# coin-or/Ipopt

Measured on AMD Instinct MI355X. Metric: KKT factor+solve GFLOP/s (1 numeric LDL^T factorisation + 2 solves per Ipopt iteration), higher is better.
Workload: dtype f64; 1 GPU; synth_1e6; kkt_dim=1000000, triplet_nnz=20143342, nnz_L=230755000, ordering=nested dissection + minimum-degree leaves (own), supernodes=50052, tree_levels=110, maxfront=3260, num_neg=400000

## Files before the change

ipopt_amd/csrc/api.cpp:

```cpp
#include "../../include/mi355x_kkt.h"
#include "symbolic.h"
#include "numeric.h"
#include "launch_plan.h"
#include "matching_scaling.h"
#include "comm_shm.h"
#include "env_knobs.h"
#include <algorithm>
#include <cmath>
#include <cstdio>
#include <cstring>
#include <new>
#include <string>
#include <thread>
#include <chrono>
#include <vector>

using namespace mi355x;

struct mi355x_kkt_handle_s {
    mi355x_kkt_options opts;
    Symbolic sym;
    Numeric* num = nullptr;
    bool analysed = false, numeric_ready = false, factored = false;
    bool stats_stale = false;
// ... 435 lines not shown
        case 21: v = &S.dup_ptr; break;    case 22: v = &S.dup_src; break;    case 23: v = &S.sn_class; break;
        case 24: v = &S.rslot_ptr; break;  case 25: v = &S.rslot_idx; break;  case 26: v = &S.rslot_col; break;
        default: h->err = "get_symbolic: unknown selector"; return MI355X_KKT_FATAL;
    }
    if ((int64_t)v->size() > cap) { h->err = "get_symbolic: buffer too small"; return MI355X_KKT_FATAL; }
    if (!v->empty()) std::memcpy(out, v->data(), v->size() * sizeof(int));
    return MI355X_KKT_SUCCESS;
}

int mi355x_kkt_get_launch_plan(mi355x_kkt_handle h, int nranks, int rank, const char* what, int* out, int64_t cap, int64_t* count)
{
    if (!h || !what || !count) return MI355X_KKT_FATAL;
    if (!h->analysed) { h->err = "get_launch_plan: analyse() first"; return MI355X_KKT_FATAL; }
    if (nranks != std::max(1, h->so.nranks) || rank < 0 || rank >= nranks) { h->err = "get_launch_plan: nranks is the analysis's, 0 <= rank < nranks"; return MI355X_KKT_FATAL; }
    try {
        const LaunchPlan P = build_launch_plan(h->sym, plan_inputs_from_env(nranks, rank, nranks > 1, 0));
        if (!P.error.empty()) { h->err = P.error; return MI355X_KKT_FATAL; }
        std::vector<int> v;
        auto put = [&](std::initializer_list<long long> x) { for (long long e : x) v.push_back((int)e); };
        const std::string w(what);
        const Sched* sc = w.rfind("single.", 0) == 0 ? &P.single : w.rfind("local.", 0) == 0 ? &P.local : nullptr;
        if (w.rfind("stage", 0) == 0) { const int d = atoi(w.c_str() + 5); if (d >= 0 && d < (int)P.stage.size()) sc = &P.stage[d]; }
        const std::string field = sc ? w.substr(w.find('.') + 1) : w;
        if (sc) {
            if (field == "ptr") v = sc->ptr; else if (field == "base") put({sc->base}); else if (field == "maxm") v = sc->maxm; else if (field == "maxk") v = sc->maxk;
            else if (field == "last0") v = sc->last0; else if (field == "last1") v = sc->last1; else if (field == "allsolo") v.assign(sc->allsolo.begin(), sc->allsolo.end());
            else { h->err = "get_launch_plan: unknown schedule field"; return MI355X_KKT_FATAL; }
        } else if (w == "scalars") put({P.nlevels, P.ndepth, P.lc_levels, P.lc_nchains, P.la_any, P.grouped, P.ntfuse, P.nbig, (long long)P.stage.size()});
        else if (w == "level_list") v = P.lvl_list;
        else if (w == "tiny16") v = P.tiny16;
        else if (w == "tiny_split") v = P.tiny_split;
        else if (w == "mid_split") v = P.mid_split;
        else if (w == "big_split") v = P.big_split;
        else if (w == "lc_ptr") v = P.lc_ptr;
        else if (w == "lc_fronts") { for (const LeafLink& K : P.lc_link) v.push_back(K.s); if (P.lc_levels == 0) v.clear(); }
        else if (w == "df_runs") for (const DfRun& R : P.df_runs) put({R.lv0, R.lv1, R.tab0, R.nlev, R.nq});
        else if (w == "chain_segs") for (const ChainSeg& G : P.chain_segs) put({G.lv0, G.lv1, G.desc0, G.ndesc, G.nwg_f, G.nwg_b, G.maxtail, G.wgf0, G.wgb0});
        else if (w == "chain_links") for (const ChainLink& K : P.chl) put({K.s, K.k, K.koff, K.fi});
        else if (w == "chain_descs") for (const ChainDesc& D : P.chd) put({D.link0, D.nlinks, D.tail, D.ktot, D.s0, D.init});
        else if (w == "join") for (const JoinList& J : P.join) put({J.base, J.count, J.maxm, J.who});
        else if (w == "exchange") for (const RangeSeg& G : P.ex.rsegs) put({G.d, G.glo, G.gsz, G.aend - G.abeg, G.tend - G.tbeg});
        else if (w == "col_owner") v = P.col_owner;
        else if (w == "stat_owner") v = P.stat_owner;
        else { h->err = "get_launch_plan: unknown array"; return MI355X_KKT_FATAL; }
        *count = (int64_t)v.size();
        if (out) { if ((int64_t)v.size() > cap) { h->err = "get_launch_plan: buffer too small"; return MI355X_KKT_FATAL; } std::copy(v.begin(), v.end(), out); }
        return MI355X_KKT_SUCCESS;
    } catch (...) { h->err = "get_launch_plan: unexpected exception"; return MI355X_KKT_FATAL; }
}

int mi355x_kkt_profile(mi355x_kkt_handle h, int reps, double* ms, int* launches, int capacity)
{
    if (!h || !ms || !launches) return MI355X_KKT_FATAL;
    if (!h->numeric_ready || !h->factored) { h->err = "profile: factor() first"; return MI355X_KKT_FATAL; }
    if (capacity < MI355X_KKT_KERNEL_COUNT) { h->err = "profile: capacity too small"; return MI355X_KKT_FATAL; }
    try { if (!h->num->profile(reps > 0 ? reps : 1, ms, launches)) { h->err = h->num->error(); return MI355X_KKT_FATAL; } return MI355X_KKT_SUCCESS; }
    catch (...) { h->err = "profile: unexpected exception"; return MI355X_KKT_FATAL; }
}

int mi355x_kkt_debug_clocks(mi355x_kkt_handle h, unsigned long long* out128)
{
    if (!h || !h->numeric_ready) return MI355X_KKT_FATAL;
    try { return h->num->debug_clocks(out128) ? 0 : MI355X_KKT_FATAL; } catch (...) { return MI355X_KKT_FATAL; }
}

int mi355x_kkt_debug_pivots(mi355x_kkt_handle h, double* dinv, double* doff, int* ptype, int* lperm)
// ... 88 lines not shown
```

ipopt_amd/csrc/kernels_fronts.hip.inc:

```
template <int TS>
__device__ __forceinline__ void publish_col(double* buf, const double (&t)[TS][TS], const int row0, const int jl)
{
#pragma unroll
    for (int b = 0; b < TS; ++b)
        if (jl == b) {
#pragma unroll
            for (int a = 0; a < TS; ++a) { double v = t[a][b]; asm volatile("" : "+v"(v)); buf[row0 + a] = v; }
        }
}

#ifdef MI355X_PIVSTAT
__device__ unsigned long long g_fstat[32];
__device__ unsigned long long g_dt[16], g_dtacc[16];
__device__ unsigned long long g_pivstat[16];
#ifdef MI355X_PIVSTAT_COUNT
#define PIVSTAT(i) do { if (threadIdx.x == 0) atomicAdd(&g_pivstat[i], 1ull); } while (0)
#else
#define PIVSTAT(i) do { } while (0)
#endif
#else
#define PIVSTAT(i) do { } while (0)
#endif

__device__ __forceinline__ double fast_rcp(double d)
// ... 689 lines not shown
    }
#pragma unroll
    for (int sl = 0; sl < 2; ++sl) {
        const int r = wrow[sl];
        if (r >= 0 && r < m) {
#pragma unroll
            for (int g = 0; g < 4; ++g) { const int c = l4 + 4 * g; if (c < k) F[pk(r, c)] = wacc[sl][g]; }
        }
    }
    __syncthreads();
    {
        int q = 0;
        for (int tc = 0; tc < ntl; ++tc)
            for (int ti = max(tc, 1); ti < ntl; ++ti, ++q) {
                if ((q & 3) != wave) continue;
                v4f64_ acc = (v4f64_){0.0, 0.0, 0.0, 0.0};
                const int ri = 16 * ti + l15, rc = 16 * tc + l15;
#pragma unroll
                for (int t = 0; t < 4; ++t) {
                    const int p = 4 * t + l4;
                    const double av = (ri < m && p < k) ? F[pk(min(ri, m - 1), p)] * dinv_s[min(p, 15)] : 0.0;
                    const double bv = (rc < m && rc >= k && p < k) ? F[pk(min(max(rc, p), m - 1), p)] : 0.0;
                    acc = __builtin_amdgcn_mfma_f64_16x16x4f64(av, bv, acc, 0, 0, 0);
                }
                const int cc = 16 * tc + l15;
#pragma unroll
                for (int g = 0; g < 4; ++g) { const int rr = 16 * ti + l4 + 4 * g; if (rr < m && cc >= k && rr >= cc) F[pk(rr, cc)] -= acc[g]; }
            }
    }
    __syncthreads();
    return true;
}

template <int J> __device__ __forceinline__ void fast16_step_masked(double (&a)[16], double& rsave, const int l15, const bool on)
{
    const double t = a[J];
    const double d = bcast16<J>(t);
    const double ri = on ? fast_rcp(d) : 0.0;
    rsave = (on && l15 == J) ? ri : rsave;
    const double l = on ? t * ri : 0.0;
    rank1_dpp16<J>(a, t, l);
    a[J] = on ? l : t;
}
__device__ __forceinline__ void st_coh(double* p, double v);
__device__ __forceinline__ void st_coh(int* p, int v);
__device__ __forceinline__ void st_tagged(v2d* p, const double v, const double ep) { const v2d m = (v2d){v, ep}; asm volatile("global_store_dwordx4 %0, %1, off sc1" :: "v"(p), "v"(m) : "memory"); }
__device__ __forceinline__ void ld_tagged_row16(const v2d* p, v2d (&r)[16])
{
    asm volatile("global_load_dwordx4 %0, %16, off sc1\n\tglobal_load_dwordx4 %1, %16, off offset:256 sc1\n\tglobal_load_dwordx4 %2, %16, off offset:512 sc1\n\tglobal_load_dwordx4 %3, %16, off offset:768 sc1\n\t"
                 "global_load_dwordx4 %4, %16, off offset:1024 sc1\n\tglobal_load_dwordx4 %5, %16, off offset:1280 sc1\n\tglobal_load_dwordx4 %6, %16, off offset:1536 sc1\n\tglobal_load_dwordx4 %7, %16, off offset:1792 sc1\n\t"
                 "global_load_dwordx4 %8, %16, off offset:2048 sc1\n\tglobal_load_dwordx4 %9, %16, off offset:2304 sc1\n\tglobal_load_dwordx4 %10, %16, off offset:2560 sc1\n\tglobal_load_dwordx4 %11, %16, off offset:2816 sc1\n\t"
                 "global_load_dwordx4 %12, %16, off offset:3072 sc1\n\tglobal_load_dwordx4 %13, %16, off offset:3328 sc1\n\tglobal_load_dwordx4 %14, %16, off offset:3584 sc1\n\tglobal_load_dwordx4 %15, %16, off offset:3840 sc1\n\t"
                 "s_waitcnt vmcnt(0)"
                 : "=&v"(r[0]), "=&v"(r[1]), "=&v"(r[2]), "=&v"(r[3]), "=&v"(r[4]), "=&v"(r[5]), "=&v"(r[6]), "=&v"(r[7]), "=&v"(r[8]), "=&v"(r[9]), "=&v"(r[10]), "=&v"(r[11]), "=&v"(r[12]), "=&v"(r[13]), "=&v"(r[14]), "=&v"(r[15])
                 : "v"(p) : "memory");
}
__device__ __forceinline__ bool df_wait_expired(const DevView& V, const int spins)
{
    if (spins > (1 << 22) || ((spins & 1023) == 0 && __hip_atomic_load(&V.qstat[6], __ATOMIC_RELAXED, __HIP_MEMORY_SCOPE_AGENT) != 0)) { V.qstat[6] = 1; V.qstat[4] = 1; return true; }
    return false;
}
template <bool DF>
__device__ __forceinline__ void front_dpp16_body(const DevView& V, double (&Fs)[4][16 * 17], int (&relS)[4][16], const int list_off, const int nfronts, const int quad, const int top_mode, const int no_strict_behind, const int epoch)
{
    const int lane = threadIdx.x, g = lane >> 4, li = lane & 15;
    const int f = 4 * quad + g;
// ... 570 lines not shown
```

ipopt_amd/csrc/launch_plan.cpp:

```cpp
#include "launch_plan.h"
#include "env_knobs.h"
#include <algorithm>
#include <cstdio>
#include <map>

namespace mi355x {

PlanInputs plan_inputs_from_env(int nranks, int rank, bool multi, int verbose)
{
    PlanInputs in;
    in.nranks = nranks; in.rank = rank; in.multi = multi; in.verbose = verbose;
    in.chain_solve = !knob_disabled("chain_solve"); in.fuse_dt = !knob_disabled("fuse_dt"); in.fastpiv = !knob_disabled("fastpiv");
    in.asm_pull = !knob_disabled("asm_pull"); in.leafchain = !knob_disabled("leafchain"); in.front_df = !knob_disabled("front_df");
    in.tfuse = !knob_disabled("tfuse"); in.fuse_upd = !knob_disabled("fuse_upd"); in.selfasm = !knob_disabled("selfasm");
    in.grouped = !knob_disabled("grouped"); in.xcd_tiles = !knob_disabled("xcd_tiles"); in.lookahead = !knob_disabled("lookahead");
    in.pair_solve = !knob_disabled("pair_solve"); in.p1_small = !knob_disabled("p1_small");
    in.la_wgs = (int)std::max(1ll, knob_int("la_wgs", in.la_wgs));
    in.la_min_nt = (int)std::max(3ll, knob_int("la_min_nt", in.la_min_nt));
    in.la_min_tiles = knob_int("la_min_tiles", in.la_min_tiles);
    in.grp_rbw_max = (int)std::max(1ll, knob_int("grp_rbw_max", in.grp_rbw_max));
    in.chain_solve_maxc = (int)std::max(1ll, knob_int("chain_solve_maxc", in.chain_solve_maxc));
    in.fuse_dt_maxwg = (int)knob_int("fuse_dt_maxwg", in.fuse_dt_maxwg);
    knob_tune("fastpiv_floor", &in.fastpiv_floor);
    return in;
}

static int order_of(const Symbolic& Sy, int s) { return Sy.sn_rowptr[s + 1] - Sy.sn_rowptr[s]; }
static int cols_of(const Symbolic& Sy, int s) { return Sy.sn_colptr[s + 1] - Sy.sn_colptr[s]; }
static int nchild(const Symbolic& Sy, int s) { return Sy.child_ptr[s + 1] - Sy.child_ptr[s]; }
static int tri_tiles(int nt) { const int t = nt * (nt + 1) / 2; return nt >= 12 ? (t + 7) / 8 * 8 : t; }
static int schur_tiles64(const Symbolic& Sy, int s)
{
    const int nt = (order_of(Sy, s) - cols_of(Sy, s) + 63) / 64;
    return Sy.grp_rem[s] > 0 ? nt * ((Sy.grp_rem[s] + 63) / 64) : nt * (nt + 1) / 2;
}
static int schur_tiles(const Symbolic& Sy, int s)
{
    const int nt = (order_of(Sy, s) - cols_of(Sy, s) + 127) / 128;
    return Sy.grp_rem[s] > 0 ? nt * ((Sy.grp_rem[s] + 127) / 128) : tri_tiles(nt);
}
static size_t front_lds(size_t m, size_t k, size_t maxm)
{
    const size_t ld = m | 1, ldi = k | 1;
    return (std::max(m * (m + 1) / 2, k * ld + k * ldi) + 4 * maxm + 3 * k) * sizeof(double) + 2 * k * sizeof(int) + 64;
}
static bool same_range(const Symbolic& Sy, int a, int b) { return Sy.sn_owner[a] < 0 && Sy.sn_owner[b] < 0 && Sy.sn_glo[a] == Sy.sn_glo[b] && Sy.sn_gsz[a] == Sy.sn_gsz[b]; }
static bool crosses(const Symbolic& Sy, int c) { const int pa = Sy.sn_parent[c]; return pa >= 0 && Sy.sn_owner[pa] < 0 && !same_range(Sy, c, pa); }

ExchangeLayout exchange_layout(const Symbolic& Sy, int ndepth)
// ... 23 lines not shown
        }
        X.aend[d] = X.arena_doubles; X.tend[d] = X.toprhs_doubles;
    }
    return X;
}

void comm_plan(const Symbolic& Sy, int nranks, int rank, bool range_local, std::vector<int>& out)
{
    const int ndepth = std::max(1, Sy.num_gdepths);
    const ExchangeLayout X = exchange_layout(Sy, ndepth);
    auto rec = [&](int what, int d, int colour, int gsz, long long count, int dtype) { out.push_back(what); out.push_back(d); out.push_back(colour); out.push_back(gsz); out.push_back((int)std::min<long long>(count, 0x7fffffffll)); out.push_back(dtype); };
    if (range_local)
        for (int d = 0; d < ndepth; ++d) {
            bool partial = false; int color = -1;
            for (const RangeSeg& sg : X.rsegs) if (sg.d == d && sg.gsz < nranks) { partial = true; if (sg.glo <= rank && rank < sg.glo + sg.gsz) color = sg.glo; }
            if (partial) rec(0, d, color, 0, 0, 1);
        }
    auto step = [&](int d, int what) {
        if (range_local) {
            for (const RangeSeg& sg : X.rsegs) {
                if (sg.d != d || !(sg.glo <= rank && rank < sg.glo + sg.gsz)) continue;
                const long long cnt = what == 1 ? sg.aend - sg.abeg : sg.tend - sg.tbeg;
                if (cnt > 0) rec(what, d, sg.gsz >= nranks ? -2 : sg.glo, sg.gsz, cnt, 0);
            }
        } else {
            const long long cnt = what == 1 ? X.aend[d] - X.abeg[d] : X.tend[d] - X.tbeg[d];
            if (cnt > 0) rec(what, d, -2, nranks, cnt, 0);
        }
    };
    for (int d = ndepth - 1; d >= 0; --d) step(d, 1);
    rec(2, 0, -2, nranks, 8, 1);
    for (int d = ndepth - 1; d >= 0; --d) step(d, 3);
    if (Sy.n > 0) rec(4, 0, -2, nranks, Sy.n, 0);
}

LaunchPlan build_launch_plan(const Symbolic& Sy, const PlanInputs& in)
{
    LaunchPlan P;
    const int NL = Sy.num_levels, NS = Sy.num_sn;
    const bool multi = in.multi;
    P.nlevels = NL;
    auto bucket0 = [&](int lv, int fc) { return Sy.level_ptr[(size_t)lv * FC_COUNT + fc]; };
    auto pool_remap = [&](long long lin) {
        if (in.pool_cut.empty()) return lin;
        const size_t i = (size_t)(std::upper_bound(in.pool_cut.begin(), in.pool_cut.end(), lin) - in.pool_cut.begin()) - 1; return lin + in.pool_delta[i]; };
    P.panel_off.resize(NS); P.cb_off.resize(NS);
    for (int sn = 0; sn < NS; ++sn) {
        P.panel_off[sn] = pool_remap(Sy.panel_off[sn]);
        P.cb_off[sn] = pool_remap(Sy.l_doubles + Sy.cb_off[sn]) - Sy.l_doubles;
    }
    std::vector<int>& L = P.lvl_list;
    L.assign(Sy.level_sn.begin(), Sy.level_sn.end());
    std::vector<char> solve_entry;
    auto in_sched = [&](int which, int s) {
        if (which == 0) return true;
        if (which == 1) return Sy.sn_owner[s] == in.rank;
        return Sy.sn_owner[s] < 0 && Sy.sn_glo[s] <= in.rank && in.rank < Sy.sn_glo[s] + Sy.sn_gsz[s] && Sy.sn_gdepth[s] == which - 2;
    };
    auto build_sched = [&](Sched& sc, int which) {
        sc.ptr.assign((size_t)NL * FC_COUNT + 1, 0); sc.base = which == 0 ? 0 : (int)L.size();
        sc.maxm.assign(NL, 0); sc.maxk.assign(NL, 0); sc.tiles.assign(NL, 0); sc.tiles64.assign(NL, 0);
        std::vector<std::vector<int>> bucket((size_t)NL * FC_COUNT);
        for (int s = 0; s < NS; ++s) {
            if (!in_sched(which, s)) continue;
            const int lv = Sy.sn_level[s];
            bucket[(size_t)lv * FC_COUNT + Sy.sn_class[s]].push_back(s);
// ... 250 lines not shown
    auto build_groups = [&](GrpSched& G, int which) {
        for (auto* v : {&G.g0, &G.g1, &G.split, &G.nrb, &G.tiles64, &G.tiles, &G.la1, &G.la2, &G.p1t, &G.la3, &G.nsplit}) v->assign(NL, 0);
        if (!P.grouped) return;
        std::vector<std::vector<int>> at(NL);
        for (int sn = 0; sn < NS; ++sn) if (Sy.sn_class[sn] == FC_BIG && Sy.grp_rem[sn] == 0 && in_sched(which, sn)) {
            int first = sn;
            for (int j = Sy.grp_pos[sn]; j > 0; --j) first = Sy.alias_child[first];
            if (Sy.sn_level[first] >= Sy.grp_cut_level) at[Sy.sn_level[first]].push_back(sn);
        }
        int ng = 0;
        for (int lv = 0; lv < NL; ++lv) {
            std::stable_sort(at[lv].begin(), at[lv].end(), [&](int a, int b) { return order_of(Sy, a) < order_of(Sy, b); });
            G.g0[lv] = (int)L.size();
            int nsmall = 0;
            for (int sn : at[lv]) {
                L.push_back(sn); ++ng;
                const int mu = upd_rows(sn), nt = (mu + 127) / 128;
                G.nrb[lv] = std::max(G.nrb[lv], (mu + 63) / 64);
                if (order_of(Sy, sn) <= 1024) { ++nsmall; G.tiles64[lv] = std::max(G.tiles64[lv], schur_tiles64(Sy, sn)); continue; }
                G.tiles[lv] = std::max(G.tiles[lv], schur_tiles(Sy, sn));
                G.la1[lv] = std::max(G.la1[lv], split_of[sn] ? 2 * nt - 1 : tri_tiles(nt));
                if (split_of[sn]) {
                    G.la2[lv] = std::max(G.la2[lv], ((nt - 2) * (nt - 1) / 2 + 7) / 8 * 8);
                    const int n64 = (mu + 63) / 64; int c = 0; for (int tc = 0; tc < 4 && tc < n64; ++tc) c += n64 - tc; G.p1t[lv] = std::max(G.p1t[lv], c); ++G.nsplit[lv];
                } else G.la3[lv] = std::max(G.la3[lv], tri_tiles(nt));
            }
            G.split[lv] = nsmall; G.g1[lv] = (int)L.size();
        }
        if (in.verbose) fprintf(stderr, "[mi355x_kkt] grouped schedule%s: %d chain groups factored in one launch each (tree levels >= %d)\n",
                                which == 0 ? "" : (which == 1 ? " (own subtrees)" : " (replicated fronts of one exchange step)"), ng, Sy.grp_cut_level);
    };
    P.grp.assign(multi ? 1 + P.ndepth : 1, GrpSched());
    for (size_t i = 0; i < P.grp.size(); ++i) build_groups(P.grp[i], multi ? 1 + (int)i : 0);
    std::vector<char> tfuse_of(NS, 0);
    std::vector<int> asmcut_of(NS, 0);
    if (!multi && in.tfuse)
        for (int sn = 0; sn < NS; ++sn) {
            if (Sy.sn_class[sn] != FC_BIG || Sy.grp_rem[sn] != 0) continue;
            int first = sn;
            for (int j = 0; j < Sy.grp_pos[sn]; ++j) first = Sy.alias_child[first];
            if (Sy.alias_child[first] >= 0 || upd_rows(sn) <= 0 || nchild(Sy, first) > 96) continue;
            tfuse_of[sn] = 1; ++P.ntfuse;
            asmcut_of[first] = order_of(Sy, first) - upd_rows(sn);
        }
    if (in.verbose) fprintf(stderr, "[mi355x_kkt] contribution blocks formed by their update (not assembled): %d of %d big fronts\n", P.ntfuse, Sy.num_big);
    P.fmeta.resize(L.size()); P.asm_fast_ok.assign(L.size(), 0); P.asmcut.assign(L.size(), 0);
    for (size_t q = 0; q < L.size(); ++q) {
        const int sn = L[q];
        FrontMeta& M = P.fmeta[q];
        int nside = 0;
        for (int c = Sy.child_ptr[sn]; c < Sy.child_ptr[sn + 1]; ++c) if (Sy.child_idx[c] != Sy.alias_child[sn]) ++nside;
        P.asm_fast_ok[q] = (Sy.alias_child[sn] >= 0 && nside == 0) ? 1 : (Sy.alias_child[sn] < 0 ? (nside <= 6 ? std::max(nside, 1) : 0) : 0);
        M.tfuse = tfuse_of[sn]; M.asmcut = asmcut_of[sn];
        M.s = sn; M.c0 = Sy.sn_colptr[sn]; M.k = cols_of(Sy, sn); M.r0 = Sy.sn_rowptr[sn]; M.m = order_of(Sy, sn);
        M.aq0 = Sy.acolptr[M.c0]; M.aq1 = Sy.acolptr[M.c0 + M.k]; M.ch0 = Sy.child_ptr[sn]; M.ch1 = Sy.child_ptr[sn + 1]; M.alias = Sy.alias_child[sn] >= 0 ? 1 : 0;
        M.ldp = Sy.sn_ldp[sn]; M.ldt = Sy.sn_ldt[sn];
        M.panel_off = P.panel_off[sn]; M.cb_off = P.cb_off[sn]; M.minv_off = Sy.minv_off[sn];
        M.cv = Sy.cv_off[sn]; M.wb = Sy.wb_off[sn]; M.gpart = Sy.gpart_off[sn];
        M.gbase = gbase_of[sn]; M.gpos = Sy.grp_pos[sn]; M.grem = Sy.grp_rem[sn]; M.gcols = gcols_of[sn]; M.split = split_of[sn]; M.ttab = ttab_of[sn]; M.ttab2 = ttab2_of[sn];
        M.selfasm = (Sy.sn_class[sn] == FC_BIG && selfasm(sn)) ? 1 : 0; M.bigidx = bigidx_of[sn];
        M.solo = (Sy.alias_child[sn] >= 0 && nchild(Sy, sn) == 1) ? 1 : ((Sy.alias_child[sn] < 0 && nchild(Sy, sn) == 0) ? 2 : 0);
        P.asmcut[q] = (M.selfasm && !M.asmcut) ? -1 : M.asmcut;
        if (q < solve_entry.size() && solve_entry[q] && !Sy.solve_group) {
            M.gbase += M.gpos; M.gpos = 0; M.grem = 0; M.gcols = M.k;
        }
    }
// ... 97 lines not shown
```

ipopt_amd/csrc/launch_plan.h:

```cpp
#pragma once
#include "symbolic.h"
#include "kernel_tables.h"
#include <cstddef>
#include <string>
#include <vector>

namespace mi355x {

struct PlanInputs {
    int nranks = 1, rank = 0;
    bool multi = false;
    int verbose = 0;
    bool chain_solve = true, fuse_dt = true, fastpiv = true, asm_pull = true, leafchain = true, front_df = true, tfuse = true, fuse_upd = true,
         selfasm = true, grouped = true, xcd_tiles = true, lookahead = true, pair_solve = true, p1_small = true;
    int la_wgs = 1 << 20, la_min_nt = 8, grp_rbw_max = 8, chain_solve_maxc = 128, fuse_dt_maxwg = 448;
    long long la_min_tiles = 4000;
    double fastpiv_floor = 1e-4;
    std::vector<long long> pool_cut, pool_delta;
};
PlanInputs plan_inputs_from_env(int nranks, int rank, bool multi, int verbose);

struct Sched { std::vector<int> ptr; int base = 0; std::vector<int> maxm, maxk, tiles, tiles64, last0, last1; std::vector<char> allsolo; };
struct GrpSched { std::vector<int> g0, g1, split, nrb, tiles64, tiles, la1, la2, p1t, la3, nsplit; };
struct ChainSeg { int lv0, lv1, desc0, ndesc, nwg_f, nwg_b, maxtail, wgf0, wgb0; };
struct JoinList { int base = 0, count = 0, maxm = 0, who = -1; };
struct RangeSeg { int d, glo, gsz; long long abeg, aend, tbeg, tend; };
struct DfRun { int lv0, lv1, tab0, nlev, nq; };

struct ExchangeLayout {
    std::vector<long long> aoff, troff;
    std::vector<long long> abeg, aend, tbeg, tend;
    std::vector<RangeSeg> rsegs;
    long long arena_doubles = 0, toprhs_doubles = 0;
};
ExchangeLayout exchange_layout(const Symbolic& Sy, int ndepth);
void comm_plan(const Symbolic& S, int nranks, int rank, bool range_local, std::vector<int>& out6);

struct LaunchPlan {
    int nlevels = 0;
    std::vector<int> lvl_list;
    Sched single;
    int ndepth = 1;
    Sched local; std::vector<Sched> stage;
    std::vector<JoinList> join;
    ExchangeLayout ex;
    std::vector<int> tiny16, tiny_split, mid_split, big_split, part_tiles[2];
    std::vector<size_t> mid_lds, reg_lds;
    std::vector<int> wave_kmax, wave_mmax, wave_mmin;
    bool pair_solve = true;
    std::vector<ChainSeg> chain_segs; std::vector<int> seg_at_lv0, seg_at_lv1;
    std::vector<char> in_seg;
    std::vector<ChainLink> chl; std::vector<ChainDesc> chd; std::vector<int> chwait, wgf, wgb;
    int ntailflags = 0, ndots = 0;
    std::vector<int> la_tiles1, la_tiles2; std::vector<char> la_full;
    bool la_any = false;
    std::vector<int> tile_tab;
    std::vector<char> lv_asm_skip;
    std::vector<int> lv_narrow_tiles;
    bool grouped = false;
    std::vector<GrpSched> grp;
    std::vector<char> asm_fast_ok; std::vector<int> asmcut;
    int ntfuse = 0, nbig = 0;
    std::string error;
    int lc_levels = 0, lc_nchains = 0;
    std::vector<int> lc_ptr; std::vector<LeafLink> lc_link;
    std::vector<DfRun> df_runs; std::vector<int> df_run_at; std::vector<DfLevel> df_tab; std::vector<long long> cbt_off; long long cbt_len = 0;
    std::vector<FrontMeta> fmeta; std::vector<ChildMeta> cmeta; std::vector<GroupLink> gtab; std::vector<int> relinv;
    std::vector<long long> panel_off, cb_off;
    std::vector<int> stat_owner, col_owner;
};
LaunchPlan build_launch_plan(const Symbolic& Sy, const PlanInputs& in);

}
```

ipopt_amd/csrc/numeric.hip:

```cpp
#include <hip/hip_runtime.h>
#include <rccl/rccl.h>
#include <dlfcn.h>
#include <cstdio>
#include <cstring>
#include <cmath>
#include <chrono>
#include <vector>
#include <thread>
#include <map>
#include <string>
#include <algorithm>
#include "numeric.h"
#include "launch_plan.h"
#include "env_knobs.h"
#include "matching_scaling.h"

namespace mi355x {

#define HIPCHK(call) do { hipError_t e_ = (call); if (e_ != hipSuccess) { \
    err_ = std::string(#call) + ": " + hipGetErrorString(e_); return false; } } while (0)

enum KernelKind { KK_GATHER_SCALE = 0, KK_FRONT_WAVE, KK_FRONT_LDS64, KK_FRONT_LDS128, KK_BIG_ASSEMBLE, KK_BIG_DIAG, KK_BIG_TRSM,
                  KK_BIG_SCHUR, KK_STATS, KK_SOLVE_PERM, KK_FWD_WAVE, KK_FWD_LDS, KK_FWD_BIG, KK_BWD_WAVE, KK_BWD_LDS, KK_BWD_BIG, KK_FWD_BIG_UPD, KK_BWD_BIG_DOT, KK_COUNT };
#define DBGSTAMP(slot) do { if (V.dbg && blockIdx.x == 0 && blockIdx.y == 0 && threadIdx.x == 0) { V.dbg[2 * (slot)] = clock64(); V.dbg[2 * (slot) + 1] = wall_clock64(); } } while (0)
// ... 551 lines not shown
        V.tvals = tv;
        V.rslot_len = (int)Sy.rslot_idx.size();
        if (!dalloc(&V.arv, Sy.rslot_idx.size()) || !dalloc(&V.aval, Sy.nnz_a) || !dalloc(&V.scale, Sy.n) || !dalloc(&V.scale2, Sy.n) || !dalloc(&V.rowmax, Sy.n) ||
            !dalloc(&V.wbuf, (size_t)Sy.wbuf_doubles) || !dalloc(&V.minv, (size_t)Sy.minv_doubles) ||
            !dalloc(&V.dinv, Sy.n) || !dalloc(&V.doff, Sy.n) || !dalloc(&V.ptype, Sy.n) || !dalloc(&V.lperm, Sy.n) ||
            !dalloc(&V.fstat, Sy.num_sn) || !dalloc(&V.xw, Sy.n) || !dalloc(&V.ybuf, Sy.n) || !dalloc(&V.zb, Sy.n) || !dalloc(&V.bw, Sy.n) || !dalloc(&V.xacc, Sy.n) || !dalloc(&V.cvec, (size_t)Sy.cvec_doubles) || !dalloc(&V.gpart, (size_t)Sy.gpart_doubles) ||
            !dalloc(&d_stats, 12) || !dalloc(&V.colfail, Sy.n) || !dalloc(&V.zpiv, Sy.n) || !dalloc(&V.cnorm, Sy.n) ||
            !dalloc(&V.sflag_d, Sy.num_sn) || !dalloc(&V.sflag_p, Sy.num_sn) || !dalloc(&V.sflag_s, 4 * (size_t)Sy.num_sn) || !dalloc(&V.tcnt, Sy.num_sn) || !dalloc(&V.apfail, Sy.num_sn) || !dalloc(&V.sepoch, 4)) return false;
        V.qstat = d_stats + 4;
        lap("device allocations");
        if (opt.scaling >= 3 && !d_user_scale) { HIPCHK(hipMalloc((void**)&d_user_scale, std::max<size_t>(Sy.n, 1) * sizeof(double))); allocs.push_back(d_user_scale); }
        else if (opt.scaling == 2 && !d_user_scale) opt.scaling = 1;
        V.cb = V.L + Sy.l_doubles;
        V.arena = nullptr; V.top_rhs = nullptr; V.rank = opt.rank; V.dbg = nullptr;
        if (knob_trace("clocks")) { if (!dalloc(&V.dbg, 128)) return false; }
        if (multi) { if (!dalloc(&V.arena, (size_t)P.ex.arena_doubles) || !dalloc(&V.top_rhs, (size_t)P.ex.toprhs_doubles)) return false; }
        V.pivtol = opt.pivtol; V.pivtol2 = std::max(opt.pivtol, opt.pivtolmax); V.small = opt.small; V.n = Sy.n; V.nnz_a = Sy.nnz_a; V.nsn = Sy.num_sn; V.xcd_affine = knob_disabled("xcd_affine") ? 0 : 1;
        la_ev.assign(1 + P.grp.size(), LaEvents());
        for (size_t i = 0; i < la_ev.size(); ++i) {
            const std::vector<int>& la2 = i == 0 ? P.la_tiles2 : P.grp[i - 1].la2;
            la_ev[i].A.assign(la2.size(), nullptr); la_ev[i].B.assign(la2.size(), nullptr);
            for (size_t lv = 0; lv < la2.size(); ++lv) if (la2[lv] > 0) {
                HIPCHK(hipEventCreateWithFlags(&la_ev[i].A[lv], hipEventDisableTiming)); HIPCHK(hipEventCreateWithFlags(&la_ev[i].B[lv], hipEventDisableTiming)); }
        }
        HIPCHK(hipFuncSetAttribute((const void*)k_big_diag_reg<4>, hipFuncAttributeMaxDynamicSharedMemorySize, 160 * 1024));
        HIPCHK(hipFuncSetAttribute((const void*)(k_big_diag_reg<4, 1024>), hipFuncAttributeMaxDynamicSharedMemorySize, 160 * 1024));
        HIPCHK(hipFuncSetAttribute((const void*)(k_front_reg<64, 2>), hipFuncAttributeMaxDynamicSharedMemorySize, 160 * 1024));
        HIPCHK(hipFuncSetAttribute((const void*)(k_front_reg<64, 4>), hipFuncAttributeMaxDynamicSharedMemorySize, 160 * 1024));
        HIPCHK(hipFuncSetAttribute((const void*)(k_front_reg<64, 8>), hipFuncAttributeMaxDynamicSharedMemorySize, 160 * 1024));
        HIPCHK(hipFuncSetAttribute((const void*)(k_front_reg<256, 8>), hipFuncAttributeMaxDynamicSharedMemorySize, 160 * 1024));
        HIPCHK(hipFuncSetAttribute((const void*)(k_front_reg<256, 6>), hipFuncAttributeMaxDynamicSharedMemorySize, 160 * 1024));
        HIPCHK(hipFuncSetAttribute((const void*)(k_front_reg<256, 8, true>), hipFuncAttributeMaxDynamicSharedMemorySize, 160 * 1024));
        HIPCHK(hipFuncSetAttribute((const void*)(k_front_reg<256, 6, true, 4>), hipFuncAttributeMaxDynamicSharedMemorySize, 160 * 1024));
        HIPCHK(hipFuncSetAttribute((const void*)k_big_trsm<false>, hipFuncAttributeMaxDynamicSharedMemorySize, 160 * 1024));
        HIPCHK(hipFuncSetAttribute((const void*)k_big_trsm<true>, hipFuncAttributeMaxDynamicSharedMemorySize, 160 * 1024));
        HIPCHK(hipFuncSetAttribute((const void*)k_big_diag_trsm, hipFuncAttributeMaxDynamicSharedMemorySize, 160 * 1024));
        HIPCHK(hipFuncSetAttribute((const void*)k_grp_fused, hipFuncAttributeMaxDynamicSharedMemorySize, 160 * 1024));
        HIPCHK(hipFuncSetAttribute((const void*)k_big_assemble2, hipFuncAttributeMaxDynamicSharedMemorySize, 158 * 1024));
        HIPCHK(hipDeviceSynchronize());
        lap("kernel attributes, zero fills landed");
        ready = true;
        if (keep && comm_kind == 2) make_subcomms();
        return true;
    }

    static size_t trsm_lds(int kk) { return trsm_lds_bytes(kk, false); }
    static int schur_grid(int tiles) { return SCHUR_GM == 2 ? 16 * ((tiles + 7) / 8) : tiles; }
    int grid1d(long long n) const { long long g = (n + 255) / 256; return (int)std::min<long long>(std::max<long long>(g, 1), 2048); }


    bool launch_bucket(int lv, int fc, int b0, int b1, int top_mode, int mm, int kk, int tiles, int tiles64) {
        const int nb = b1 - b0;
        const size_t rl = P.reg_lds[(size_t)lv * FC_COUNT + fc];
        if (fc == FC_WAVE) {
            const bool sg = b0 == S->level_ptr[(size_t)lv * FC_COUNT + FC_WAVE];
            const int nt = sg ? P.tiny_split[lv] : 0;
            int fl = top_mode;
            if (V.fastpiv && P.wave_mmin[lv] <= 16) {
                const int n16 = sg ? P.tiny16[lv] : nb;
                if (n16 > 0) { LAUNCH(KK_FRONT_WAVE, k_front_dpp16, dim3((n16 + 3) / 4), dim3(64), 0, stream, V, b0, n16, top_mode, (optimistic && n16 == nb) ? 1 : 0); fl |= 2; }
                if (optimistic && n16 == nb) return true;
            }
            if (nt > 0) LAUNCH(KK_FRONT_WAVE, (k_front_reg<64, 2>), dim3(nt), dim3(64), rl, stream, V, b0, fl);
            if (nb - nt > 0) LAUNCH(KK_FRONT_WAVE, (k_front_reg<64, 4>), dim3(nb - nt), dim3(64), rl, stream, V, b0 + nt, fl);
        } else if (fc == FC_LDS64) {
            LAUNCH(KK_FRONT_LDS64, (k_front_reg<64, 8>), dim3(nb), dim3(64), rl, stream, V, b0, top_mode);
        } else if (fc == FC_LDS128) {
            const int nm = (b0 == S->level_ptr[(size_t)lv * FC_COUNT + FC_LDS128]) ? P.mid_split[lv] : 0;
            const int fl = top_mode | (V.fastpiv ? 2 : 0);
            if (V.fastpiv) {
                if (nm > 0) LAUNCH(KK_FRONT_LDS128, (k_front_reg<256, 6, true, 4>), dim3(nm), dim3(256), P.mid_lds[lv], stream, V, b0, top_mode);
                if (nb - nm > 0) LAUNCH(KK_FRONT_LDS128, (k_front_reg<256, 8, true>), dim3(nb - nm), dim3(256), rl, stream, V, b0 + nm, top_mode);
            }
            if (nm > 0) LAUNCH(KK_FRONT_LDS128, (k_front_reg<256, 6>), dim3(nm), dim3(256), P.mid_lds[lv], stream, V, b0, fl);
            if (nb - nm > 0) LAUNCH(KK_FRONT_LDS128, (k_front_reg<256, 8>), dim3(nb - nm), dim3(256), rl, stream, V, b0 + nm, fl);
        } else {
            const bool single = (b0 == S->level_ptr[(size_t)lv * FC_COUNT + FC_BIG]) && !multi;
            if ((single || multi) && P.grouped && lv >= S->grp_cut_level) {
                if (!(single && P.lv_asm_skip[lv])) launch_assemble(mm, nb, b0, top_mode);
                return launch_groups(lv, top_mode ? 1 + grp_step : 0);
            }
            if (!single) { const bool sm = mm <= 640; return launch_big(lv, b0, sm ? b1 : b0, b1, top_mode, mm, kk, sm ? tiles64 : 0, sm ? 0 : tiles, false); }
            return launch_big(lv, b0, b0 + P.big_split[lv], b1, top_mode, mm, kk, P.part_tiles[0][lv], P.part_tiles[1][lv], true);
        }
        return true;
    }
    bool launch_groups(int lv, int gi) {
        const GrpSched& G = P.grp[gi]; const LaEvents& E = la_ev[1 + gi];
        const int b0 = G.g0[lv], b1 = G.g1[lv], bs = b0 + G.split[lv];
        if (b1 == b0) return true;
        {
            int rbw = 1;
            while (rbw < knobs.grp_rbw_max && (b1 - b0) * (4 + (G.nrb[lv] + rbw - 1) / rbw) > 256) rbw *= 2;
            const int nrbw = (G.nrb[lv] + rbw - 1) / rbw;
            const int st = ((b1 - b0) * (4 + nrbw) <= 256) ? 1 : 0;
            const size_t lds = std::max(diag_lds_bytes(64, 64), GRP_DB_BYTES + trsm_lds_bytes(64, st != 0));
            LAUNCH(KK_BIG_DIAG, k_grp_fused, dim3(b1 - b0, 4 + nrbw), dim3(256), lds, stream, V, b0, st, rbw, 0);
        }
        if (bs > b0 && G.tiles64[lv] > 0) LAUNCH(KK_BIG_SCHUR, k_big_schur64, dim3(G.tiles64[lv], bs - b0), dim3(256), 0, stream, V, b0, 0);
        if (b1 == bs) return true;
        const int nb = b1 - bs;
        if (la_pending) { HIPCHK(hipStreamWaitEvent(stream, la_last, 0)); la_pending = false; }
        if (G.la2[lv] > 0) {
            if (knobs.p1_small && G.la1[lv] * nb <= 512) {
                LAUNCH(KK_BIG_SCHUR, k_big_schur_p1, dim3(G.p1t[lv], nb), dim3(1024), 0, stream, V, bs);
                if (G.nsplit[lv] < nb) LAUNCH(KK_BIG_SCHUR, k_big_schur, dim3(schur_grid(G.la3[lv]), nb), dim3(SCHUR_NT), 0, stream, V, bs, 4, 0, 0);
            } else LAUNCH(KK_BIG_SCHUR, k_big_schur, dim3(schur_grid(G.la1[lv]), nb), dim3(SCHUR_NT), 0, stream, V, bs, 1, 0, 0);
            HIPCHK(hipEventRecord(E.A[lv], stream));
            HIPCHK(hipStreamWaitEvent(stream2, E.A[lv], 0));
            launch_part2(bs, nb, G.la2[lv]);
            HIPCHK(hipEventRecord(E.B[lv], stream2));
            la_last = E.B[lv]; la_pending = true;
        } else if (G.tiles[lv] > 0) LAUNCH(KK_BIG_SCHUR, k_big_schur, dim3(schur_grid(G.tiles[lv]), nb), dim3(SCHUR_NT), 0, stream, V, bs, 0, 0, 0);
// ... 947 lines not shown
```

Before: 9733 GFLOP/s.

## Add single-workgroup LDS-resident front kernel for small big-class supernodes

Adds k_front_wg, a 512-thread kernel that assembles, factors (16-column MFMA blocks with pivot checks), writes L/contribution blocks and inverts the diagonal block of a FC_BIG front entirely in LDS. The launch plan partitions each level's big fronts into eligible ones (order up to 192, at most 64 columns, not aliased or grouped), which use this kernel, and the rest, which stay on the multi-kernel big path. The aim is to cut launches and global round-trips for small big-class fronts. The cost is a new code path gated on the optimistic mode, packed-triangular LDS indexing, and another kernel whose numerics must match the existing path.

```diff
diff --git a/ipopt_amd/csrc/api.cpp b/ipopt_amd/csrc/api.cpp
--- a/ipopt_amd/csrc/api.cpp
+++ b/ipopt_amd/csrc/api.cpp
@@ -491,6 +491,7 @@
         else if (w == "tiny_split") v = P.tiny_split;
         else if (w == "mid_split") v = P.mid_split;
         else if (w == "big_split") v = P.big_split;
+        else if (w == "front_wg") for (int lv = 0; lv < P.nlevels; ++lv) put({P.wg0[lv], P.wg1[lv], P.rest0[lv], P.rest1[lv], P.rest_split[lv], P.wg_maxm[lv], P.wg_maxk[lv]});
         else if (w == "lc_ptr") v = P.lc_ptr;
         else if (w == "lc_fronts") { for (const LeafLink& K : P.lc_link) v.push_back(K.s); if (P.lc_levels == 0) v.clear(); }
         else if (w == "df_runs") for (const DfRun& R : P.df_runs) put({R.lv0, R.lv1, R.tab0, R.nlev, R.nq});
diff --git a/ipopt_amd/csrc/kernels_fronts.hip.inc b/ipopt_amd/csrc/kernels_fronts.hip.inc
--- a/ipopt_amd/csrc/kernels_fronts.hip.inc
+++ b/ipopt_amd/csrc/kernels_fronts.hip.inc
@@ -745,6 +745,186 @@
     return true;
 }
 
+constexpr int FRONT_WG_NT = 512;
+static size_t front_wg_lds_bytes(size_t m, size_t k) { return (std::max(m * (m + 1) / 2, k * (k | 1)) + 272 + 128) * sizeof(double) + 16; }
+template <int NT>
+__global__ __launch_bounds__(NT) void k_front_wg(DevView V, int list_off)
+{
+    extern __shared__ __attribute__((aligned(16))) char smem_raw[];
+    constexpr int NW = NT / 64;
+    const int tid = threadIdx.x, lane = tid & 63, wave = tid >> 6, l15 = lane & 15, l4 = lane >> 4;
+    const FrontMeta M = V.fmeta[list_off + blockIdx.x];
+    const int s = M.s, c0 = M.c0, k = M.k, m = M.m;
+    const int npk = m * (m + 1) / 2, ldi = k | 1;
+    double* F      = reinterpret_cast<double*>(smem_raw);
+    double* Xs     = F + max(npk, k * ldi);
+    double* dinv_s = Xs + 272;
+    double* cmv    = dinv_s + 64;
+    int*    shflag = reinterpret_cast<int*>(cmv + 64);
+    auto pk = [m](int i, int c) { return c * m - ((c * (c - 1)) >> 1) + (i - c); };
+    for (int idx = tid; idx < npk; idx += NT) F[idx] = 0.0;
+    if (tid == 0) { shflag[0] = 0; shflag[1] = 0; }
+    __syncthreads();
+    for (int q = M.aq0 + tid; q < M.aq1; q += NT) { const int pos = V.apos[q]; const int i = pos % m, c = pos / m; F[pk(i, c)] += V.aval[q]; }
+    __syncthreads();
+    {
+        int* relS = reinterpret_cast<int*>(Xs);
+        for (int cp = M.ch0; cp < M.ch1; ++cp) {
+            const ChildMeta* Cp = V.cmeta + cp;
+            const int mc = Cp->mc, ldt = Cp->ldt;
+            const double* C = V.cb + Cp->cb_off;
+            const int* relg = V.rel + Cp->relbase;
+            const unsigned d = (unsigned)(mc + 1), inv = 0xFFFFFFFFu / d + 1u;
+            const int npr = (mc + 1) >> 1, total = npr * (mc + 1);
+            for (int a = tid; a < mc; a += NT) relS[a] = relg[a];
+            auto decode = [&](int e, int& a, int& b) -> bool {
+                const int pr = (int)__umulhi((unsigned)e, inv), q = e - pr * (mc + 1);
+                const bool second = q >= mc - pr;
+                b = second ? mc - 1 - pr : pr;
+                a = second ? b + (q - (mc - pr)) : pr + q;
+                return e < total && !(second && 2 * pr == mc - 1);
+            };
+            __syncthreads();
+            constexpr int U = 8;
+            for (int base = 0; base < total; base += NT * U) {
+                double cvv[U];
+#pragma unroll
+                for (int u = 0; u < U; ++u) { int a, b; cvv[u] = decode(base + tid + NT * u, a, b) ? C[a + (size_t)b * ldt] : 0.0; }
+#pragma unroll
+                for (int u = 0; u < U; ++u) { int a, b; if (decode(base + tid + NT * u, a, b)) F[pk(relS[a], relS[b])] += cvv[u]; }
+            }
+            __syncthreads();
+        }
+    }
+    for (int c = tid >> 4; c < 64; c += NT / 16) {
+        const int part = tid & 15;
+        double mx = 0.0;
+        if (c < k) for (int i = part; i < m; i += 16) mx = fmax(mx, fabs(F[pk(max(i, c), min(i, c))]));
+        mx = fmax(mx, dpp_f64<0xB1>(mx)); mx = fmax(mx, dpp_f64<0x4E>(mx)); mx = fmax(mx, dpp_f64<0x141>(mx)); mx = fmax(mx, dpp_f64<0x140>(mx));
+        if (part == 0) cmv[c] = (c < k) ? fmax(mx, V.cnorm[c0 + c]) : 0.0;
+    }
+    __syncthreads();
+    const double cmx = wave_max_all(cmv[lane]);
+    const double zmax = fmax(V.small, ZERO_REL * cmx);
+    const double gmax = 1.0 / fmax(fmax(V.pivtol, V.pivtol2), V.fastu);
+    const int nbk = (k + 15) >> 4, ntl = (m + 15) >> 4;
+    int neg = 0;
+    bool ok = true;
+    for (int b = 0; b < nbk && ok; ++b) {
+        const int c16 = 16 * b, kb = min(16, k - c16);
+        if (wave == 0) {
+            const int row = c16 + l15;
+            double a[16], w[16], rsave = 1.0;
+#pragma unroll
+            for (int c = 0; c < 16; ++c) {
+                const int rr = min(row, m - 1), cc = min(c16 + c, m - 1);
+                const double v = F[pk(max(rr, cc), min(rr, cc))];
+                a[c] = (row < m && c16 + c < m) ? v : ((l15 == c) ? 1.0 : 0.0);
+                w[c] = 0.0;
+            }
+            asm volatile("s_waitcnt lgkmcnt(0)" ::: "memory");
+#define MI_STEP(j) if (j < kb) fast16_step<j>(a, w, rsave, l15);
+            MI_STEP(0) MI_STEP(1) MI_STEP(2) MI_STEP(3) MI_STEP(4) MI_STEP(5) MI_STEP(6) MI_STEP(7)
+            MI_STEP(8) MI_STEP(9) MI_STEP(10) MI_STEP(11) MI_STEP(12) MI_STEP(13) MI_STEP(14) MI_STEP(15)
+#undef MI_STEP
+            double gm = 0.0;
+#pragma unroll
+            for (int c = 0; c < 15; ++c) gm = fmax(gm, (c < kb && l15 > c) ? fabs(a[c]) : 0.0);
+            const bool mine = l15 < kb;
+            bool bad = __ballot(gm > gmax) != 0ull;
+            bad |= __ballot(mine && !(fabs(rsave) * zmax < 1.0)) != 0ull;
+            neg += __popcll(__ballot(mine && l4 == 0 && rsave < 0.0));
+            double x[4];
+#pragma unroll
+            for (int q = 0; q < 4; ++q) x[q] = (l15 == 4 * q + l4) ? 1.0 : 0.0;
+#define MI_INV(j) if (j + 1 < kb) fast16_inv<j>(a, x, l15, kb);
+            MI_INV(0) MI_INV(1) MI_INV(2) MI_INV(3) MI_INV(4) MI_INV(5) MI_INV(6) MI_INV(7) MI_INV(8) MI_INV(9) MI_INV(10) MI_INV(11) MI_INV(12) MI_INV(13) MI_INV(14)
+#undef MI_INV
+            if (bad) { if (lane == 0) shflag[0] = 1; }
+            else {
+#pragma unroll
+                for (int q = 0; q < 4; ++q) Xs[l15 + (4 * q + l4) * 17] = x[q];
+                if (l4 == 0 && mine) dinv_s[row] = rsave;
+                if (lane == 0) shflag[1] = neg;
+                if (l4 == 0 && row < m) {
+#pragma unroll
+                    for (int c = 0; c < 16; ++c) {
+                        if (c < kb) { if (l15 > c) F[pk(row, c16 + c)] = w[c]; }
+                        else if (l15 >= c) F[pk(row, c16 + c)] = a[c];
+                    }
+                }
+            }
+        }
+        __syncthreads();
+        if (shflag[0]) { ok = false; break; }
+        {
+            bool big = false;
+            for (int t = b + 1 + wave; t < ntl; t += NW) {
+                const int r = 16 * t + l15;
+                v4f64_ acc = (v4f64_){0.0, 0.0, 0.0, 0.0};
+#pragma unroll
+                for (int u = 0; u < 4; ++u) {
+                    const int p = 4 * u + l4;
+                    const double av = (p < kb && l15 < kb) ? Xs[l15 + p * 17] : 0.0;
+                    const double bv = (r < m && p < kb) ? F[pk(min(r, m - 1), c16 + min(p, kb - 1))] : 0.0;
+                    acc = __builtin_amdgcn_mfma_f64_16x16x4f64(av, bv, acc, 0, 0, 0);
+                }
+#pragma unroll
+                for (int g = 0; g < 4; ++g) {
+                    const int c = l4 + 4 * g;
+                    if (c < kb && r < m) { big |= fabs(acc[g] * dinv_s[c16 + c]) > gmax; F[pk(r, c16 + c)] = acc[g]; }
+                }
+            }
+            if (__ballot(big) != 0ull && lane == 0) shflag[0] = 1;
+        }
+        __syncthreads();
+        if (shflag[0]) { ok = false; break; }
+        {
+            int q = 0;
+            for (int tc = (kb == 16) ? b + 1 : b; tc < ntl; ++tc)
+                for (int ti = max(tc, b + 1); ti < ntl; ++ti, ++q) {
+                    if (q % NW != wave) continue;
+                    v4f64_ acc = (v4f64_){0.0, 0.0, 0.0, 0.0};
+                    const int ri = 16 * ti + l15, rc = 16 * tc + l15;
+#pragma unroll
+                    for (int t = 0; t < 4; ++t) {
+                        const int p = 4 * t + l4, col = c16 + min(p, kb - 1);
+                        const double av = (ri < m && p < kb) ? F[pk(min(ri, m - 1), col)] * dinv_s[col] : 0.0;
+                        const double bv = (rc < m && rc >= c16 + kb && p < kb) ? F[pk(min(max(rc, col), m - 1), col)] : 0.0;
+                        acc = __builtin_amdgcn_mfma_f64_16x16x4f64(av, bv, acc, 0, 0, 0);
+                    }
+                    const int cc = 16 * tc + l15;
+#pragma unroll
+                    for (int g = 0; g < 4; ++g) { const int rr = 16 * ti + l4 + 4 * g; if (rr < m && cc >= c16 + kb && rr >= cc) F[pk(rr, cc)] -= acc[g]; }
+                }
+        }
+        __syncthreads();
+    }
+    if (!ok) { if (tid == 0) { V.fstat[s] = make_int4(0, 0, 0, 0); V.qstat[4] = 1; } return; }
+    double* Lg = V.L + M.panel_off;
+    const size_t ldp = (size_t)M.ldp, ldt = (size_t)M.ldt;
+    for (int c = wave; c < k; c += NW) {
+        const double di = dinv_s[c];
+        for (int i = lane; i < m; i += 64) Lg[i + (size_t)c * ldp] = (i > c) ? F[pk(i, c)] * di : 0.0;
+    }
+    for (int jj = tid; jj < k; jj += NT) { V.dinv[c0 + jj] = dinv_s[jj]; V.doff[c0 + jj] = 0.0; V.ptype[c0 + jj] = 1; V.lperm[c0 + jj] = jj; }
+    double* Cg = V.cb + M.cb_off;
+    for (int c = k + wave; c < m; c += NW)
+        for (int i = c + lane; i < m; i += 64) Cg[(i - k) + (size_t)(c - k) * ldt] = F[pk(i, c)];
+    if (tid == 0) { V.fstat[s] = make_int4(shflag[1], 0, 0, 0); atomicAdd(&V.qstat[3], 1); }
+    constexpr int E = 4096 / NT;
+    double tmp[E];
+#pragma unroll
+    for (int e = 0; e < E; ++e) { const int idx = tid + e * NT; const int i = idx % k, c = idx / k; tmp[e] = (idx < k * k && i > c) ? F[pk(i, c)] * dinv_s[c] : 0.0; }
+    __syncthreads();
+#pragma unroll
+    for (int e = 0; e < E; ++e) { const int idx = tid + e * NT; const int i = idx % k, c = idx / k; if (idx < k * k) F[i + c * ldi] = tmp[e]; }
+    __syncthreads();
+    invert_unit_lower<NT>(F, ldi, k);
+    double* Mg = V.minv + M.minv_off;
+    for (int idx = tid; idx < k * k; idx += NT) { const int i = idx % k, c = idx / k; Mg[idx] = (i > c) ? F[i + c * ldi] : (i == c ? 1.0 : 0.0); }
+}
+
 template <int J> __device__ __forceinline__ void fast16_step_masked(double (&a)[16], double& rsave, const int l15, const bool on)
 {
     const double t = a[J];
diff --git a/ipopt_amd/csrc/launch_plan.cpp b/ipopt_amd/csrc/launch_plan.cpp
--- a/ipopt_amd/csrc/launch_plan.cpp
+++ b/ipopt_amd/csrc/launch_plan.cpp
@@ -14,7 +14,9 @@
     in.asm_pull = !knob_disabled("asm_pull"); in.leafchain = !knob_disabled("leafchain"); in.front_df = !knob_disabled("front_df");
     in.tfuse = !knob_disabled("tfuse"); in.fuse_upd = !knob_disabled("fuse_upd"); in.selfasm = !knob_disabled("selfasm");
     in.grouped = !knob_disabled("grouped"); in.xcd_tiles = !knob_disabled("xcd_tiles"); in.lookahead = !knob_disabled("lookahead");
-    in.pair_solve = !knob_disabled("pair_solve"); in.p1_small = !knob_disabled("p1_small");
+    in.pair_solve = !knob_disabled("pair_solve"); in.p1_small = !knob_disabled("p1_small"); in.front_wg = !knob_disabled("front_wg");
+    in.front_wg_partial = knob_int("front_wg_partial", in.front_wg_partial ? 1 : 0) != 0;
+    in.front_wg_maxm = (int)std::min<long long>(FRONT_WG_MAXM, std::max(0ll, knob_int("front_wg_maxm", in.front_wg_maxm)));
     in.la_wgs = (int)std::max(1ll, knob_int("la_wgs", in.la_wgs));
     in.la_min_nt = (int)std::max(3ll, knob_int("la_min_nt", in.la_min_nt));
     in.la_min_tiles = knob_int("la_min_tiles", in.la_min_tiles);
@@ -104,6 +106,12 @@
     rec(2, 0, -2, nranks, 8, 1);
     for (int d = ndepth - 1; d >= 0; --d) step(d, 3);
     if (Sy.n > 0) rec(4, 0, -2, nranks, Sy.n, 0);
+}
+
+bool front_wg_eligible(const Symbolic& Sy, int sn, int maxm)
+{
+    return Sy.sn_class[sn] == FC_BIG && order_of(Sy, sn) <= maxm && cols_of(Sy, sn) <= FRONT_WG_MAXK &&
+           Sy.alias_child[sn] < 0 && Sy.grp_pos[sn] == 0 && Sy.grp_rem[sn] == 0;
 }
 
 LaunchPlan build_launch_plan(const Symbolic& Sy, const PlanInputs& in)
@@ -420,6 +428,21 @@
     };
     P.grp.assign(multi ? 1 + P.ndepth : 1, GrpSched());
     for (size_t i = 0; i < P.grp.size(); ++i) build_groups(P.grp[i], multi ? 1 + (int)i : 0);
+    for (auto* v : {&P.wg0, &P.wg1, &P.wg_maxm, &P.wg_maxk, &P.rest0, &P.rest1, &P.rest_split, &P.rest_tiles[0], &P.rest_tiles[1]}) v->assign(NL, 0);
+    for (int lv = 0; lv < NL && !multi && in.front_wg; ++lv) {
+        if (P.grouped && lv >= Sy.grp_cut_level) continue;
+        std::vector<int> wg, rest;
+        for (int q = bucket0(lv, FC_BIG); q < bucket0(lv, FC_BIG + 1); ++q) (front_wg_eligible(Sy, L[q], in.front_wg_maxm) ? wg : rest).push_back(L[q]);
+        if (wg.empty() || (!rest.empty() && !in.front_wg_partial)) continue;
+        P.wg0[lv] = (int)L.size(); L.insert(L.end(), wg.begin(), wg.end()); P.wg1[lv] = (int)L.size();
+        for (int sn : wg) { P.wg_maxm[lv] = std::max(P.wg_maxm[lv], order_of(Sy, sn)); P.wg_maxk[lv] = std::max(P.wg_maxk[lv], cols_of(Sy, sn)); }
+        P.rest0[lv] = (int)L.size(); L.insert(L.end(), rest.begin(), rest.end()); P.rest1[lv] = (int)L.size();
+        for (int sn : rest) {
+            const int h = order_of(Sy, sn) <= 1024 ? 0 : 1;
+            if (h == 0) ++P.rest_split[lv];
+            P.rest_tiles[h][lv] = std::max(P.rest_tiles[h][lv], h == 0 ? schur_tiles64(Sy, sn) : schur_tiles(Sy, sn));
+        }
+    }
     std::vector<char> tfuse_of(NS, 0);
     std::vector<int> asmcut_of(NS, 0);
     if (!multi && in.tfuse)
diff --git a/ipopt_amd/csrc/launch_plan.h b/ipopt_amd/csrc/launch_plan.h
--- a/ipopt_amd/csrc/launch_plan.h
+++ b/ipopt_amd/csrc/launch_plan.h
@@ -12,8 +12,10 @@
     bool multi = false;
     int verbose = 0;
     bool chain_solve = true, fuse_dt = true, fastpiv = true, asm_pull = true, leafchain = true, front_df = true, tfuse = true, fuse_upd = true,
-         selfasm = true, grouped = true, xcd_tiles = true, lookahead = true, pair_solve = true, p1_small = true;
+         selfasm = true, grouped = true, xcd_tiles = true, lookahead = true, pair_solve = true, p1_small = true, front_wg = true;
     int la_wgs = 1 << 20, la_min_nt = 8, grp_rbw_max = 8, chain_solve_maxc = 128, fuse_dt_maxwg = 448;
+    bool front_wg_partial = true;
+    int front_wg_maxm = 192;
     long long la_min_tiles = 4000;
     double fastpiv_floor = 1e-4;
     std::vector<long long> pool_cut, pool_delta;
@@ -36,6 +38,9 @@
 ExchangeLayout exchange_layout(const Symbolic& Sy, int ndepth);
 void comm_plan(const Symbolic& S, int nranks, int rank, bool range_local, std::vector<int>& out6);
 
+constexpr int FRONT_WG_MAXM = 192, FRONT_WG_MAXK = 64;
+bool front_wg_eligible(const Symbolic& Sy, int sn, int maxm);
+
 struct LaunchPlan {
     int nlevels = 0;
     std::vector<int> lvl_list;
@@ -45,6 +50,7 @@
     std::vector<JoinList> join;
     ExchangeLayout ex;
     std::vector<int> tiny16, tiny_split, mid_split, big_split, part_tiles[2];
+    std::vector<int> wg0, wg1, wg_maxm, wg_maxk, rest0, rest1, rest_split, rest_tiles[2];
     std::vector<size_t> mid_lds, reg_lds;
     std::vector<int> wave_kmax, wave_mmax, wave_mmin;
     bool pair_solve = true;
diff --git a/ipopt_amd/csrc/numeric.hip b/ipopt_amd/csrc/numeric.hip
--- a/ipopt_amd/csrc/numeric.hip
+++ b/ipopt_amd/csrc/numeric.hip
@@ -607,6 +607,7 @@
         HIPCHK(hipFuncSetAttribute((const void*)(k_front_reg<256, 6>), hipFuncAttributeMaxDynamicSharedMemorySize, 160 * 1024));
         HIPCHK(hipFuncSetAttribute((const void*)(k_front_reg<256, 8, true>), hipFuncAttributeMaxDynamicSharedMemorySize, 160 * 1024));
         HIPCHK(hipFuncSetAttribute((const void*)(k_front_reg<256, 6, true, 4>), hipFuncAttributeMaxDynamicSharedMemorySize, 160 * 1024));
+        HIPCHK(hipFuncSetAttribute((const void*)k_front_wg<FRONT_WG_NT>, hipFuncAttributeMaxDynamicSharedMemorySize, 160 * 1024));
         HIPCHK(hipFuncSetAttribute((const void*)k_big_trsm<false>, hipFuncAttributeMaxDynamicSharedMemorySize, 160 * 1024));
         HIPCHK(hipFuncSetAttribute((const void*)k_big_trsm<true>, hipFuncAttributeMaxDynamicSharedMemorySize, 160 * 1024));
         HIPCHK(hipFuncSetAttribute((const void*)k_big_diag_trsm, hipFuncAttributeMaxDynamicSharedMemorySize, 160 * 1024));
@@ -654,6 +655,11 @@
             if ((single || multi) && P.grouped && lv >= S->grp_cut_level) {
                 if (!(single && P.lv_asm_skip[lv])) launch_assemble(mm, nb, b0, top_mode);
                 return launch_groups(lv, top_mode ? 1 + grp_step : 0);
+            }
+            if (single && optimistic && P.wg1[lv] > P.wg0[lv]) {
+                LAUNCH(KK_BIG_DIAG, k_front_wg<FRONT_WG_NT>, dim3(P.wg1[lv] - P.wg0[lv]), dim3(FRONT_WG_NT), front_wg_lds_bytes(P.wg_maxm[lv], P.wg_maxk[lv]), stream, V, P.wg0[lv]);
+                if (P.rest1[lv] == P.rest0[lv]) return true;
+                return launch_big(lv, P.rest0[lv], P.rest0[lv] + P.rest_split[lv], P.rest1[lv], top_mode, mm, kk, P.rest_tiles[0][lv], P.rest_tiles[1][lv], true);
             }
             if (!single) { const bool sm = mm <= 640; return launch_big(lv, b0, sm ? b1 : b0, b1, top_mode, mm, kk, sm ? tiles64 : 0, sm ? 0 : tiles, false); }
             return launch_big(lv, b0, b0 + P.big_split[lv], b1, top_mode, mm, kk, P.part_tiles[0][lv], P.part_tiles[1][lv], true);
```

New measurement: 9587 GFLOP/s. 0.985x the previous value.
